# TJUMMG/OCPG

Measured on AMD Instinct MI355X. Metric: clips/sec fwd+bwd (5x384x640, R101), higher is better.
Workload: dtype bf16

## Files before the change

### include/ocpg_hip.h

```cpp
#ifndef OCPG_HIP_H
#define OCPG_HIP_H
#include <stdint.h>

#ifdef __cplusplus
extern "C" {
#endif

int ocpg_msda_fwd_f32(const float* value, const int64_t* shapes, const int64_t* level_start,
                      const float* loc, const float* attn,
                      int N, int S, int M, int D, int L, int Lq, int P,
                      float* out, const int64_t* shapes_host, void* stream);
int ocpg_msda_fwd_f64(const double* value, const int64_t* shapes, const int64_t* level_start,
                      const double* loc, const double* attn,
                      int N, int S, int M, int D, int L, int Lq, int P,
                      double* out, void* stream);

int ocpg_msda_bwd_f32(const float* value, const int64_t* shapes, const int64_t* level_start,
                      const float* loc, const float* attn, const float* grad_out,
                      int N, int S, int M, int D, int L, int Lq, int P,
                      float* grad_value, float* grad_loc, float* grad_attn,
                      const int64_t* shapes_host, void* stream);
int ocpg_msda_bwd_value_f32(const float* loc, const float* attn, const float* grad_out,
                            int N, int S, int M, int D, int L, int Lq, int P,
                            float* grad_value, const int64_t* shapes_host, void* stream);
// ... 6 lines not shown
                            int N, int S, int M, int D, int L, int Lq, int P,
                            float* out, float* loc_out, float* attn_out, void* stream);
int ocpg_msda_fused_bwd_qproj_f32(const float* value, const int64_t* shapes, const int64_t* level_start,
                                  const float* loc, const float* attn, const float* grad_out,
                                  int N, int S, int M, int D, int L, int Lq, int P,
                                  float* grad_qproj, void* stream);
int ocpg_msda_bwd_value_sel_f32(const float* loc, const float* attn, const float* grad_out,
                                int N, int S, int M, int D, int L, int Lq, int P,
                                float* grad_value, const int64_t* shapes_host, int* sel_state, void* stream);
int ocpg_msda_bwd_f64(const double* value, const int64_t* shapes, const int64_t* level_start,
                      const double* loc, const double* attn, const double* grad_out,
                      int N, int S, int M, int D, int L, int Lq, int P,
                      double* grad_value, double* grad_loc, double* grad_attn, void* stream);

int ocpg_bn_act_fwd(const void* x, const float* scale, const float* shift, const void* skip, void* y,
                    long long n_outer, int C, long long inner, int relu, int dtype, void* stream);
int ocpg_bn_act_bwd(const void* gy, const void* y, const float* scale, void* gx, void* gskip,
                    long long n_outer, int C, long long inner, int relu, int dtype, void* stream);

int ocpg_gemm_dgrad_bn_tile(long long M, int N, int K);
int ocpg_gemm_dgrad_bn(const void* a, const void* w, const void* c, const void* mask, const float* scale, void* out, void* out_skip,
                       long long M, int N, int K, int dtype, int tile, void* stream);

int ocpg_win_attn_fwd(const void* qkv, const float* biasT, const int* region, float scale, int BW, int NW, int N, int H,
                      int head_dim, void* out, float* lse, int dtype, void* stream);
int ocpg_win_attn_bwd(const void* qkv, const float* bias, const float* biasT, const int* region, float scale, int BW, int NW,
                      int N, int H, int head_dim, const void* out, const void* dout, const float* lse, void* dqkv, float* Dbuf,
                      float* dbiasT, int dtype, void* stream);

int ocpg_win_attn_bwd_mfma(const void* qkv, const float* bias, const float* biasT, const int* region, float scale, int BW, int NW, int N,
                           int H, int head_dim, const void* out, const void* dout, const float* lse, void* dqkv, float* Dbuf, void* dS,
                           int dtype, void* stream);

int ocpg_dynmask_fwd_f32(const float* feats, const float* params, const float* refpix, int BT, int Q, int C, int H, int W,
                         int stride, float* out, float* pre1, void* stream);

int ocpg_dynmask_bwd_pre_f32(const float* dout, const float* pre1, const float* params, int BT, int Q, int C, int H, int W,
                             int stride, float* dpre, float* part, float* w0d, void* stream);
int ocpg_dynmask_bwd_fin_f32(const float* part, const float* params, const float* refpix, const float* dw0, int BT, int Q, int C,
                             int H, int W, float* dparams, float* dref, void* stream);

int ocpg_im2col3x3_nhwc(const void* x, int N, int H, int W, int C, int stride, int dil, void* cols, int dtype, void* stream);
int ocpg_col2im3x3_nhwc(const void* dcols, int N, int H, int W, int C, int stride, int dil, void* dx, int dtype, void* stream);

int ocpg_conv3x3_mfma_fwd(const void* x, const void* w, const float* scale, const float* bias, int relu, int N, int H, int W,
                          int Cin, int Cout, int stride, void* y, void* stream);
// ... 169 lines not shown
```

### ocpg_amd/_lib.py

```python
import ctypes
import os

import torch

_HERE = os.path.dirname(os.path.abspath(__file__))
LIB_PATH = os.environ.get("OCPG_HIP_LIB") or os.path.join(_HERE, "lib", "libocpg_hip.so")
_lib = None

_i64p = ctypes.c_void_p
_vp = ctypes.c_void_p
_int = ctypes.c_int

SIGNATURES = {
    "ocpg_msda_fwd_f32": [_vp, _i64p, _i64p, _vp, _vp] + [_int] * 7 + [_vp, _vp, _vp],
    "ocpg_msda_fwd_f64": [_vp, _i64p, _i64p, _vp, _vp] + [_int] * 7 + [_vp, _vp],
    "ocpg_msda_bwd_f32": [_vp, _i64p, _i64p, _vp, _vp, _vp] + [_int] * 7 + [_vp, _vp, _vp, _vp, _vp],
    "ocpg_msda_bwd_value_f32": [_vp, _vp, _vp] + [_int] * 7 + [_vp, _vp, _vp],
    "ocpg_msda_fused_fwd_f32": [_vp, _i64p, _i64p, _vp, _vp] + [_int] * 7 + [_vp, _vp, _vp, _vp],
    "ocpg_msda_fused_bwd_qproj_f32": [_vp, _i64p, _i64p, _vp, _vp, _vp] + [_int] * 7 + [_vp, _vp],
    "ocpg_msda_bwd_value_sel_f32": [_vp, _vp, _vp] + [_int] * 7 + [_vp, _vp, _vp, _vp],
    "ocpg_msda_bwd_locattn_f32": [_vp, _i64p, _i64p, _vp, _vp, _vp] + [_int] * 7 + [_vp, _vp, _vp],
    "ocpg_msda_bwd_f64": [_vp, _i64p, _i64p, _vp, _vp, _vp] + [_int] * 7 + [_vp, _vp, _vp, _vp],
    "ocpg_bn_act_fwd": [_vp, _vp, _vp, _vp, _vp, ctypes.c_longlong, _int, ctypes.c_longlong, _int, _int, _vp],
    "ocpg_bn_act_bwd": [_vp, _vp, _vp, _vp, _vp, ctypes.c_longlong, _int, ctypes.c_longlong, _int, _int, _vp],
    "ocpg_gemm_dgrad_bn_tile": [ctypes.c_longlong, _int, _int],
    "ocpg_gemm_dgrad_bn": [_vp] * 7 + [ctypes.c_longlong, _int, _int, _int, _int, _vp],
    "ocpg_dynmask_fwd_f32": [_vp, _vp, _vp] + [_int] * 6 + [_vp, _vp, _vp],
    "ocpg_dynmask_bwd_pre_f32": [_vp, _vp, _vp] + [_int] * 6 + [_vp, _vp, _vp, _vp],
    "ocpg_dynmask_bwd_fin_f32": [_vp, _vp, _vp, _vp] + [_int] * 5 + [_vp, _vp, _vp],
    "ocpg_conv3x3_mfma_fwd": [_vp, _vp, _vp, _vp] + [_int] * 7 + [_vp, _vp],
    "ocpg_conv3x3_mfma_fwd_cols": [_vp, _vp, _vp, _vp] + [_int] * 7 + [_vp, _vp, _vp],
    "ocpg_conv3x3_mfma_dgrad": [_vp, _vp] + [_int] * 6 + [_vp, _vp],
    "ocpg_conv3x3_mfma_dgrad_masked": [_vp, _vp, _vp, _vp] + [_int] * 6 + [_vp, _vp],
    "ocpg_conv3x3_mfma_dgrad_w": [_vp, _vp, _vp, _vp] + [_int] * 6 + [_vp, _vp],
    "ocpg_conv3x3_mfma_splits": [_int] * 6,
    "ocpg_conv3x3_mfma_wgrad_splits": [_int] * 6,
    "ocpg_conv3x3_mfma_body_splits": [ctypes.c_longlong, _int, _int],
    "ocpg_conv3x3_mfma_fwd_bn_splitk": [_vp, _vp, _vp, _vp] + [_int] * 8 + [_vp, _vp, _vp],
    "ocpg_conv3x3_mfma_dgrad_w_splitk": [_vp, _vp, _vp, _vp] + [_int] * 7 + [_vp, _vp, _vp],
    "ocpg_conv3x3_mfma_wgrad": [_vp, _vp] + [_int] * 6 + [_vp, _vp],
    "ocpg_conv3x3_mfma_fwd_splitk": [_vp, _vp, _vp] + [_int] * 7 + [_vp, _vp, _int, _vp, _vp],
    "ocpg_gemm": [_vp, _vp, _vp, _vp] + [_int] * 4 + [ctypes.c_longlong] * 10 + [ctypes.c_float, ctypes.c_float, _vp],
    "ocpg_gemm_plans": [],
    "ocpg_gemm_tuned": [_vp],
    "ocpg_gemm_tune_rejected": [],
    "ocpg_gemm_set_tuning": [_int],
    "ocpg_gemm_export_picks": [_vp, ctypes.c_longlong],
    "ocpg_gemm_import_picks": [_vp, ctypes.c_longlong],
    "ocpg_window_means3x3_fwd": [_vp, ctypes.c_longlong, _int, _int, _int, _vp, _vp],
# ... 52 lines not shown
    "ocpg_colsum_partials": [_vp, ctypes.c_longlong, _int, _int, _vp, _vp],
    "ocpg_det_loss_fwd_f32": [_vp] * 7 + [ctypes.c_float] + [_int] * 5 + [_vp] * 3,
    "ocpg_det_loss_bwd_f32": [_vp] * 8 + [ctypes.c_float] + [_int] * 5 + [_vp] * 3,
    "ocpg_spectral_gate_fwd": [_vp] * 3 + [_int] * 3 + [_vp, _vp],
    "ocpg_spectral_gate_bwd": [_vp] * 4 + [_int] * 3 + [_vp, _vp, _vp],
    "ocpg_spectral_c2p": [_vp] * 3 + [_int] * 3 + [_vp, _int, _vp],
    "ocpg_spectral_p2c": [_vp] * 4 + [_int] * 3 + [_vp, _vp, _int, _vp],
    "ocpg_masked_ce_fwd_f32": [_vp] * 3 + [_int, ctypes.c_longlong, _vp, _vp],
    "ocpg_masked_ce_bwd_f32": [_vp] * 4 + [_int, ctypes.c_longlong, _vp, _vp],
    "ocpg_im2col3x3_nhwc": [_vp] + [_int] * 6 + [_vp, _int, _vp],
    "ocpg_col2im3x3_nhwc": [_vp] + [_int] * 6 + [_vp, _int, _vp],
    "ocpg_attn_smallk_fwd": [_vp, ctypes.c_longlong, _vp, ctypes.c_longlong, _vp, ctypes.c_longlong, _vp, ctypes.c_float] + [_int] * 5
                            + [ctypes.c_float, ctypes.c_ulonglong, ctypes.c_ulonglong, _vp, _vp, ctypes.c_longlong, _vp, _int, _vp],
    "ocpg_attn_smallk_bwd": [_vp, ctypes.c_longlong, _vp, ctypes.c_longlong, _vp, ctypes.c_longlong, _vp, _vp, ctypes.c_longlong, _vp,
                             ctypes.c_float] + [_int] * 5 + [ctypes.c_float, ctypes.c_ulonglong, ctypes.c_ulonglong, _vp, _vp, ctypes.c_longlong,
                                                             _vp, _vp, _int, _vp],
    "ocpg_win_attn_fwd": [_vp, _vp, _vp, ctypes.c_float] + [_int] * 5 + [_vp, _vp, _int, _vp],
    "ocpg_win_attn_bwd": [_vp, _vp, _vp, _vp, ctypes.c_float] + [_int] * 5 + [_vp] * 6 + [_int, _vp],
    "ocpg_win_attn_bwd_mfma": [_vp, _vp, _vp, _vp, ctypes.c_float] + [_int] * 5 + [_vp] * 6 + [_int, _vp],
}


_TIMING = {"on": False, "events": []}
_UNTIMED = ("ocpg_conv3x3_mfma_body_splits", "ocpg_gemm_dgrad_bn_tile", "ocpg_conv3x3_mfma_wgrad_splits", "ocpg_window_sums3x3_cl_bands", "ocpg_lfm_dft_supported", "ocpg_lfm_dft_split", "ocpg_conv3x3_mfma_splits", "ocpg_gemm_set_tuning", "ocpg_gemm_export_picks", "ocpg_gemm_import_picks", "ocpg_colsum_blocks", "ocpg_mso_wgrad_rows", "ocpg_gemm_plans", "ocpg_gemm_tuned", "ocpg_gemm_tune_rejected", "ocpg_bias_relu_dropout_bwd_slots", "ocpg_dropout_add_ln_bwd_slots", "ocpg_groupnorm_cl_work")


def enable_kernel_timing(on=True):
    _TIMING["on"] = on
    _TIMING["events"] = []


def collect_kernel_timing(work=None):
    torch.cuda.synchronize()
    out = {}
    for name, args, e0, e1 in _TIMING["events"]:
        d = out.setdefault(name, {"ms": 0.0, "n": 0, "work": 0.0, "modelled": 0})
        d["ms"] += e0.elapsed_time(e1)
        d["n"] += 1
        w = work(name, args) if work is not None else None
        if isinstance(w, tuple):
            d["work_lowp"] = d.get("work_lowp", 0.0) + (w[0] if w[1] else 0.0)
            w = w[0]
        if w is not None:
            d["work"] += w
            d["modelled"] += 1
    _TIMING["events"] = []
    _TIMING["on"] = False
# ... 39 lines not shown
        setattr(self, name, call)
        return call


def lib():
    global _lib
    if _lib is None:
        if not os.path.exists(LIB_PATH):
            raise RuntimeError(
                f"{LIB_PATH} not found: build it with `python -m ocpg_amd.csrc.build` "
                "(hipcc --offload-arch=gfx950). The HIP extension is mandatory; there is no CPU/PyTorch fallback.")
        L = ctypes.CDLL(LIB_PATH)
        for name, argtypes in SIGNATURES.items():
            fn = getattr(L, name)
            fn.argtypes = argtypes
            fn.restype = ctypes.c_int
        L.ocpg_hip_version.restype = ctypes.c_char_p
        L.ocpg_gemm_plans.restype = ctypes.c_longlong
        L.ocpg_gemm_tuned.restype = ctypes.c_longlong
        L.ocpg_gemm_tune_rejected.restype = ctypes.c_longlong
        L.ocpg_gemm_export_picks.restype = ctypes.c_longlong
        L.ocpg_gemm_set_tuning.restype = None
        L.ocpg_bias_relu_dropout_bwd_slots.restype = ctypes.c_longlong
        L.ocpg_dropout_add_ln_bwd_slots.restype = ctypes.c_longlong
        L.ocpg_groupnorm_cl_work.restype = ctypes.c_longlong
        L.ocpg_colsum_blocks.restype = ctypes.c_longlong
        _lib = _Lib(L)
    return _lib


def check(status, what):
    if status != 0:
        if status <= -1000:
            raise RuntimeError(f"{what}: invalid argument #{-status - 1000}")
        raise RuntimeError(f"{what}: HIP error {-status}")


def stream_ptr():
    return ctypes.c_void_p(torch.cuda.current_stream().cuda_stream)


def require_gpu(name, t):
    if not t.is_cuda:
        raise RuntimeError(f"{name} must be a GPU tensor: Not implemented on the CPU")
    if not t.is_contiguous():
        raise RuntimeError(f"{name} tensor has to be contiguous")
# ... 1 lines not shown
```

### ocpg_amd/csrc/fused_ln.hip

```cpp
#include <hip/hip_bf16.h>
#include <hip/hip_fp16.h>
#include <hip/hip_runtime.h>
#include <stdint.h>

#include "../../include/ocpg_hip.h"
#include "philox.h"

namespace {

using ocpg_dev::philox;

__device__ __forceinline__ void keep4(uint64_t seed, uint64_t offset, uint64_t idx4, uint32_t thr, float scale, float (&k)[4]) {
  if (thr == 0u) { k[0] = k[1] = k[2] = k[3] = 1.f; return; }
  const uint4 r = philox(make_uint2((uint32_t)seed, (uint32_t)(seed >> 32)),
                         make_uint4((uint32_t)idx4, (uint32_t)(idx4 >> 32), (uint32_t)offset, (uint32_t)(offset >> 32)));
  k[0] = r.x >= thr ? scale : 0.f; k[1] = r.y >= thr ? scale : 0.f; k[2] = r.z >= thr ? scale : 0.f; k[3] = r.w >= thr ? scale : 0.f;
}

template <typename T> struct IO;
template <> struct IO<float> {
  static __device__ __forceinline__ void load4(const float* p, float (&f)[4]) { const float4 v = *reinterpret_cast<const float4*>(p); f[0] = v.x; f[1] = v.y; f[2] = v.z; f[3] = v.w; }
  static __device__ __forceinline__ void store4(float* p, const float (&f)[4]) { *reinterpret_cast<float4*>(p) = make_float4(f[0], f[1], f[2], f[3]); }
};
template <> struct IO<__hip_bfloat16> {
  static __device__ __forceinline__ void load4(const __hip_bfloat16* p, float (&f)[4]) {
    const uint2 v = *reinterpret_cast<const uint2*>(p);
    f[0] = __uint_as_float(v.x << 16); f[1] = __uint_as_float(v.x & 0xffff0000u); f[2] = __uint_as_float(v.y << 16); f[3] = __uint_as_float(v.y & 0xffff0000u);
  }
  static __device__ __forceinline__ void store4(__hip_bfloat16* p, const float (&f)[4]) {
    uint32_t w[2];
#pragma unroll
    for (int i = 0; i < 2; ++i) {
      const __hip_bfloat16 lo = __float2bfloat16(f[2 * i]), hi = __float2bfloat16(f[2 * i + 1]);
      w[i] = (uint32_t)(*reinterpret_cast<const uint16_t*>(&lo)) | ((uint32_t)(*reinterpret_cast<const uint16_t*>(&hi)) << 16);
    }
    *reinterpret_cast<uint2*>(p) = make_uint2(w[0], w[1]);
  }
};

template <> struct IO<__half> {
// ... 199 lines not shown
  for (int g = g0; g < lpr; g += 256) {
    const int col = g * 4 * V;
    float acc[V][4];
#pragma unroll
    for (int v = 0; v < V; ++v)
#pragma unroll
      for (int j = 0; j < 4; ++j) acc[v][j] = 0.f;
    for (long long r = (long long)blockIdx.x * rpi + ro; r < R; r += (long long)gridDim.x * rpi) {
      float gv[V][4], hv[V][4], o[V][4];
      Wide<T, V>::load(gh + r * C + col, gv);
      Wide<T, V>::load(h + r * C + col, hv);
#pragma unroll
      for (int v = 0; v < V; ++v)
#pragma unroll
        for (int j = 0; j < 4; ++j) { o[v][j] = hv[v][j] > 0.f ? gv[v][j] * scale : 0.f; acc[v][j] += o[v][j]; }
      Wide<T, V>::store(ga + r * C + col, o);
    }
    float* o = dbias + ((long long)blockIdx.x * rpi + ro) * C + col;
#pragma unroll
    for (int v = 0; v < V; ++v) *reinterpret_cast<float4*>(o + 4 * v) = make_float4(acc[v][0], acc[v][1], acc[v][2], acc[v][3]);
  }
}

inline uint32_t threshold(float p) {
  if (p <= 0.f) return 0u;
  const double t = (double)p * 4294967296.0;
  return t >= 4294967295.0 ? 4294967295u : (uint32_t)t;
}

}

extern "C" {

int ocpg_dropout_add_ln_fwd(const void* x, const float* res, const float* gamma, const float* beta, long long R, int C, float eps, float p,
                            unsigned long long seed, unsigned long long offset, const unsigned long long* rng_base, int x_dtype, float* y,
                            float* mean, float* rstd, void* stream) {
  if (R < 0 || C <= 0 || C % 4 != 0 || C > 64 * 4 * NCH_MAX) return -1006;
  if (p < 0.f || p >= 1.f) return -1007;
  if (R == 0) return 0;
  if (!x || !res || !gamma || !beta) return -1001;
  if (!y || !mean || !rstd) return -1010;
  const uint32_t thr = threshold(p);
  const float scale = 1.f / (1.f - p);
  const unsigned grid = (unsigned)((R + 3) / 4);
  hipStream_t st = (hipStream_t)stream;
  if (x_dtype < 0 || x_dtype > 2) return -1008;
  const int nc = (C + 255) / 256;
#define DAL_FWD(XT_, N_) dal_fwd<XT_, N_><<<grid, 256, 0, st>>>((const XT_*)x, res, gamma, beta, R, C, eps, thr, scale, seed, offset, (const uint64_t*)rng_base, y, mean, rstd)
#define DAL_FWD_T(XT_) do { if (nc <= 1) DAL_FWD(XT_, 1); else if (nc <= 2) DAL_FWD(XT_, 2); else if (nc <= 4) DAL_FWD(XT_, 4); else DAL_FWD(XT_, 8); } while (0)
  if (x_dtype == 0) DAL_FWD_T(float); else if (x_dtype == 1) DAL_FWD_T(__hip_bfloat16); else DAL_FWD_T(__half);
  const hipError_t e = hipGetLastError();
// ... 90 lines not shown
```

### ocpg_amd/csrc/philox.h

```cpp
#pragma once
#include <hip/hip_runtime.h>
#include <stdint.h>

namespace ocpg_dev {

__device__ __forceinline__ uint4 philox(uint2 key, uint4 c) {
#pragma unroll
  for (int r = 0; r < 10; ++r) {
    const uint32_t lo0 = 0xD2511F53u * c.x, hi0 = __umulhi(0xD2511F53u, c.x);
    const uint32_t lo1 = 0xCD9E8D57u * c.z, hi1 = __umulhi(0xCD9E8D57u, c.z);
    c = make_uint4(hi1 ^ c.y ^ key.x, lo1, hi0 ^ c.w ^ key.y, lo0);
    key.x += 0x9E3779B9u;
    key.y += 0xBB67AE85u;
  }
  return c;
}

}
```

### ocpg_amd/models/deformable_transformer.py

```python
import copy

import torch
import torch.nn.functional as F
from torch import nn

from ..util.misc import fully_valid, inverse_sigmoid, mask_key, memo
from . import amp_cache
from .attention import MultiheadAttention
from .ops.functions import fused_ln_func
from .ops.modules import MSDeformAttn

FUSED_GLUE = True


def _drop_add_norm(x, res, drop, norm):
    if FUSED_GLUE and isinstance(norm, nn.LayerNorm) and norm.elementwise_affine and fused_ln_func.supported(x, res, x.shape[-1]):
        return fused_ln_func.dropout_add_layer_norm(x, res, norm, drop.p if drop.training else 0.0)
    return norm(res + drop(x))


def _ffn_hidden(src, linear1, activation, drop):
    if FUSED_GLUE and activation is F.relu and src.is_cuda and linear1.bias is not None:
        w, b = amp_cache.lookup(linear1.weight), amp_cache.lookup(linear1.bias)
        x = src
        if torch.is_autocast_enabled("cuda"):
            dt = torch.get_autocast_dtype("cuda")
            x, w, b = x.to(dt), w.to(dt), b.to(dt)
        if x.dtype == w.dtype and x.dtype in (torch.float32, torch.bfloat16, torch.float16) and w.shape[0] % 4 == 0:
            x2 = x.reshape(-1, x.shape[-1])
            splits = amp_cache._split_rows(x2.shape[0]) if amp_cache.SPLIT_K else 1
            h = fused_ln_func.LinearBiasReluDropout.apply(x2, w, b, drop.p if drop.training else 0.0, None, splits)
            return h.view(*x.shape[:-1], w.shape[0])
    return drop(activation(linear1(src)))


def _clones(module, n):
    out = []
    for _ in range(n):
        c = copy.deepcopy(module)
        for p, q in zip(module.parameters(), c.parameters()):
            if getattr(p, "_ocpg_single_use", False):
                q._ocpg_single_use = True
        out.append(c)
    return nn.ModuleList(out)


def _activation(name):
    if name == "relu":
        return F.relu
    if name == "gelu":
        return F.gelu
    if name == "glu":
        return F.glu
    raise RuntimeError(f"activation should be relu/gelu, not {name}.")


class DeformableTransformerEncoderLayer(nn.Module):
    def __init__(self, d_model=256, d_ffn=1024, dropout=0.1, activation="relu", n_levels=4, n_heads=8, n_points=4):
        super().__init__()
        self.self_attn = MSDeformAttn(d_model, n_levels, n_heads, n_points)
        self.dropout1 = nn.Dropout(dropout)
        self.norm1 = nn.LayerNorm(d_model)
        self.linear1 = amp_cache.Linear(d_model, d_ffn)
        amp_cache.mark_single_use(self.linear1)
        self.activation = _activation(activation)
        self.dropout2 = nn.Dropout(dropout)
        self.linear2 = amp_cache.Linear(d_ffn, d_model)
        amp_cache.mark_single_use(self.linear2)
        self.dropout3 = nn.Dropout(dropout)
        self.norm2 = nn.LayerNorm(d_model)

    def forward(self, src, pos, reference_points, spatial_shapes, level_start_index, padding_mask=None):
        with torch.autocast(device_type=src.device.type, enabled=False):
            q = src.float() if pos is None else src.float() + pos.float()
            attn = self.self_attn(q, reference_points, src.float(), spatial_shapes, level_start_index, padding_mask)[0]
        src = _drop_add_norm(attn, src, self.dropout1, self.norm1)
        ffn = self.linear2(_ffn_hidden(src, self.linear1, self.activation, self.dropout2))
        return _drop_add_norm(ffn, src, self.dropout3, self.norm2)


class DeformableTransformerEncoder(nn.Module):
    def __init__(self, encoder_layer, num_layers):
        super().__init__()
        self.layers = _clones(encoder_layer, num_layers)
        self.num_layers = num_layers

    @staticmethod
    def get_reference_points(spatial_shapes, valid_ratios, device):
        host = getattr(spatial_shapes, "_ocpg_host", None)
        shapes = host.tolist() if host is not None else spatial_shapes.tolist()
        per_level = []
        for lvl, (h, w) in enumerate(shapes):
            ys = torch.linspace(0.5, h - 0.5, h, dtype=torch.float32, device=device)
            xs = torch.linspace(0.5, w - 0.5, w, dtype=torch.float32, device=device)
            gy, gx = torch.meshgrid(ys, xs, indexing="ij")
            gy = gy.reshape(-1)[None] / (valid_ratios[:, None, lvl, 1] * h)
            gx = gx.reshape(-1)[None] / (valid_ratios[:, None, lvl, 0] * w)
            per_level.append(torch.stack((gx, gy), -1))
        ref = torch.cat(per_level, 1)
        return ref[:, :, None] * valid_ratios[:, None]
# ... 13 lines not shown
        self.cross_attn = MSDeformAttn(d_model, n_levels, n_heads, n_points)
        self.dropout1 = nn.Dropout(dropout)
        self.norm1 = nn.LayerNorm(d_model)
        self.self_attn = MultiheadAttention(d_model, n_heads, dropout=dropout)
        self.dropout2 = nn.Dropout(dropout)
        self.norm2 = nn.LayerNorm(d_model)
        self.linear1 = amp_cache.Linear(d_model, d_ffn)
        amp_cache.mark_single_use(self.linear1)
        self.activation = _activation(activation)
        self.dropout3 = nn.Dropout(dropout)
        self.linear2 = amp_cache.Linear(d_ffn, d_model)
        amp_cache.mark_single_use(self.linear2)
        self.dropout4 = nn.Dropout(dropout)
        self.norm3 = nn.LayerNorm(d_model)

    def forward(self, tgt, query_pos, reference_points, src, src_spatial_shapes, level_start_index, src_padding_mask=None):
        qk = tgt if query_pos is None else tgt + query_pos
        sa = self.self_attn(qk.transpose(0, 1), qk.transpose(0, 1), tgt.transpose(0, 1)).transpose(0, 1)
        tgt = _drop_add_norm(sa, tgt, self.dropout2, self.norm2)
        with torch.autocast(device_type=tgt.device.type, enabled=False):
            q = tgt.float() if query_pos is None else tgt.float() + query_pos.float()
            ca, loc, weights = self.cross_attn(q, reference_points, src.float(), src_spatial_shapes, level_start_index, src_padding_mask)
        tgt = _drop_add_norm(ca, tgt, self.dropout1, self.norm1)
        ffn = self.linear2(_ffn_hidden(tgt, self.linear1, self.activation, self.dropout3))
        return _drop_add_norm(ffn, tgt, self.dropout4, self.norm3), loc, weights


class DeformableTransformerDecoder(nn.Module):
    TOPK_SAMPLES = 30

    def __init__(self, decoder_layer, num_layers, return_intermediate=False):
        super().__init__()
        self.layers = _clones(decoder_layer, num_layers)
        self.num_layers = num_layers
        self.return_intermediate = return_intermediate
        self.compute_samples = True
        self.bbox_embed = None
        self.class_embed = None

    def forward(self, tgt, reference_points, src, src_spatial_shapes, src_level_start_index, src_valid_ratios,
                query_pos=None, src_padding_mask=None):
        out = tgt
        inter, inter_refs, inter_samples = [], [], []
        self.box_deltas = [] if self.bbox_embed is not None else None
        samples_keep = None
        for lid, layer in enumerate(self.layers):
            if reference_points.shape[-1] == 4:
# ... 144 lines not shown
```

### ocpg_amd/models/ops/functions/fused_ln_func.py

```python
import torch
from torch.autograd import Function
from torch.autograd.function import once_differentiable

from ...._lib import check, lib
from .gemm_func import mm

_DT = {torch.float32: 0, torch.bfloat16: 1, torch.float16: 2}
_calls = [0]
_active = [None]


class GraphRng:

    def __init__(self, device):
        self.state = torch.zeros(2, dtype=torch.int64, device=device)
        self.c0, self.calls = None, 0

    def __enter__(self):
        assert _active[0] is None, "nested graph captures of the dropout generator"
        self.c0 = _calls[0]
        _active[0] = self
        return self

    def __exit__(self, *exc):
        self.calls = _calls[0] - self.c0
        _calls[0] = self.c0
        _active[0] = None
        return False

    def advance(self):
# ... 43 lines not shown
              "ocpg_dropout_add_ln_fwd")
        ctx.save_for_backward(x2, res2, gamma, stats)
        ctx.meta = (float(p), seed, offset, base, x.shape, res.shape)
        return y.view(res.shape)

    @staticmethod
    @once_differentiable
    def backward(ctx, gy):
        x2, res2, gamma, stats = ctx.saved_tensors
        p, seed, offset, base, xshape, rshape = ctx.meta
        r, c = x2.shape
        gy = gy.reshape(r, c).float().contiguous()
        gx = torch.empty_like(x2) if ctx.needs_input_grad[0] else None
        gres = torch.empty_like(res2) if ctx.needs_input_grad[1] else None
        part = torch.empty((lib().ocpg_dropout_add_ln_bwd_slots(r), 2, c), dtype=torch.float32, device=x2.device)
        check(lib().ocpg_dropout_add_ln_bwd(gy.data_ptr(), x2.data_ptr(), res2.data_ptr(), gamma.data_ptr(), stats[0].data_ptr(), stats[1].data_ptr(),
                                            r, c, p, seed, offset, base, _DT[x2.dtype], None if gx is None else gx.data_ptr(),
                                            None if gres is None else gres.data_ptr(), part.data_ptr(), _st()),
              "ocpg_dropout_add_ln_bwd")
        dgb = part.sum(0)
        return (None if gx is None else gx.view(xshape), None if gres is None else gres.view(rshape), dgb[0], dgb[1], None, None, None)


class LinearBiasReluDropout(Function):
    @staticmethod
    def forward(ctx, x2, w, b, p, rng, splits):
        seed, offset, base = _unpack(rng)
        h = mm(x2, w, True)
        r, c = h.shape
        check(lib().ocpg_bias_relu_dropout_fwd(h.data_ptr(), b.data_ptr(), r, c, float(p), seed, offset, base, _DT[h.dtype], h.data_ptr(), _st()),
              "ocpg_bias_relu_dropout_fwd")
        ctx.save_for_backward(x2, w, h)
        ctx.meta = (float(p), splits)
        from ...amp_cache import deferrable
        ctx.defer_w, ctx.defer_b = deferrable(w), deferrable(b) and b.dtype == h.dtype
        return h

    @staticmethod
    @once_differentiable
    def backward(ctx, gh):
        from ...amp_cache import weight_grad
        x2, w, h = ctx.saved_tensors
        p, splits = ctx.meta
        r, c = h.shape
        gh = gh.to(h.dtype).contiguous()
        ga = torch.empty_like(h)
        slots = lib().ocpg_bias_relu_dropout_bwd_slots(r, c, _DT[h.dtype])
        part = torch.empty((slots, c), dtype=torch.float32, device=h.device)
        check(lib().ocpg_bias_relu_dropout_bwd(gh.data_ptr(), h.data_ptr(), r, c, p, _DT[h.dtype], ga.data_ptr(), part.data_ptr(), _st()),
              "ocpg_bias_relu_dropout_bwd")
        from ...amp_cache import defer_sum
        dbias = defer_sum(part, h.dtype) if (ctx.defer_b and ctx.needs_input_grad[2] and h.dtype != torch.float32) else part.sum(0).to(h.dtype)
        gx = mm(ga, w) if ctx.needs_input_grad[0] else None
        gw = weight_grad(ga, x2, ctx.defer_w) if ctx.needs_input_grad[1] else None
        return gx, gw, dbias if ctx.needs_input_grad[2] else None, None, None, None


def supported(x, res, c):
    return (x.is_cuda and x.dtype in _DT and res.dtype == torch.float32 and c % 4 == 0 and c <= 2048 and x.shape == res.shape)


def dropout_add_layer_norm(x, res, norm, p, rng=None):
    return DropoutAddLayerNorm.apply(x, res, norm.weight, norm.bias, p, norm.eps, rng)
```

Measured before the change: 60.14.

## Fuse FFN linear1 GEMM with bias-ReLU-dropout epilogue in forward and backward

Adds a bf16 MFMA GEMM kernel for K=256 transformer FFNs. In the forward pass it applies bias, ReLU and Philox dropout in the epilogue. In the backward pass it multiplies gy by w2 and applies the ReLU/dropout mask while producing per-panel bias-gradient partials. A new FeedForward autograd function wires both kernels into the encoder and decoder layers and falls back to the existing path when the shape or dtype is declined. This removes the intermediate writes and re-reads of the hidden activation and the separate elementwise kernels, at the cost of a hand-written GEMM that may be slower than the tuned library GEMM.

Measured after the change: 60.95, median of 6. 1.4% higher.

```diff
diff --git a/include/ocpg_hip.h b/include/ocpg_hip.h
--- a/include/ocpg_hip.h
+++ b/include/ocpg_hip.h
@@ -52,6 +52,12 @@
 int ocpg_gemm_dgrad_bn(const void* a, const void* w, const void* c, const void* mask, const float* scale, void* out, void* out_skip,
                        long long M, int N, int K, int dtype, int tile, void* stream);
 
+int ocpg_ffn_gemm_fwd(const void* x, const void* w1, const void* b1, void* h, long long M, int N, int K, float p, unsigned long long seed,
+                      unsigned long long offset, const unsigned long long* rng_base, int dtype, int nsplit, void* stream);
+long long ocpg_ffn_gemm_bwd_slots(long long M, int N);
+int ocpg_ffn_gemm_bwd(const void* gy, const void* w2, const void* h, void* ga, float* dbias_part, long long M, int N, int K, float p,
+                      int dtype, int nsplit, void* stream);
+
 int ocpg_win_attn_fwd(const void* qkv, const float* biasT, const int* region, float scale, int BW, int NW, int N, int H,
                       int head_dim, void* out, float* lse, int dtype, void* stream);
 int ocpg_win_attn_bwd(const void* qkv, const float* bias, const float* biasT, const int* region, float scale, int BW, int NW,
diff --git a/ocpg_amd/_lib.py b/ocpg_amd/_lib.py
--- a/ocpg_amd/_lib.py
+++ b/ocpg_amd/_lib.py
@@ -25,6 +25,9 @@
     "ocpg_bn_act_bwd": [_vp, _vp, _vp, _vp, _vp, ctypes.c_longlong, _int, ctypes.c_longlong, _int, _int, _vp],
     "ocpg_gemm_dgrad_bn_tile": [ctypes.c_longlong, _int, _int],
     "ocpg_gemm_dgrad_bn": [_vp] * 7 + [ctypes.c_longlong, _int, _int, _int, _int, _vp],
+    "ocpg_ffn_gemm_fwd": [_vp] * 4 + [ctypes.c_longlong, _int, _int, ctypes.c_float, ctypes.c_ulonglong, ctypes.c_ulonglong, _vp, _int, _int, _vp],
+    "ocpg_ffn_gemm_bwd_slots": [ctypes.c_longlong, _int],
+    "ocpg_ffn_gemm_bwd": [_vp] * 5 + [ctypes.c_longlong, _int, _int, ctypes.c_float, _int, _int, _vp],
     "ocpg_dynmask_fwd_f32": [_vp, _vp, _vp] + [_int] * 6 + [_vp, _vp, _vp],
     "ocpg_dynmask_bwd_pre_f32": [_vp, _vp, _vp] + [_int] * 6 + [_vp, _vp, _vp, _vp],
     "ocpg_dynmask_bwd_fin_f32": [_vp, _vp, _vp, _vp] + [_int] * 5 + [_vp, _vp, _vp],
@@ -123,7 +126,7 @@
 
 
 _TIMING = {"on": False, "events": []}
-_UNTIMED = ("ocpg_conv3x3_mfma_body_splits", "ocpg_gemm_dgrad_bn_tile", "ocpg_conv3x3_mfma_wgrad_splits", "ocpg_window_sums3x3_cl_bands", "ocpg_lfm_dft_supported", "ocpg_lfm_dft_split", "ocpg_conv3x3_mfma_splits", "ocpg_gemm_set_tuning", "ocpg_gemm_export_picks", "ocpg_gemm_import_picks", "ocpg_colsum_blocks", "ocpg_mso_wgrad_rows", "ocpg_gemm_plans", "ocpg_gemm_tuned", "ocpg_gemm_tune_rejected", "ocpg_bias_relu_dropout_bwd_slots", "ocpg_dropout_add_ln_bwd_slots", "ocpg_groupnorm_cl_work")
+_UNTIMED = ("ocpg_conv3x3_mfma_body_splits", "ocpg_gemm_dgrad_bn_tile", "ocpg_ffn_gemm_bwd_slots", "ocpg_conv3x3_mfma_wgrad_splits", "ocpg_window_sums3x3_cl_bands", "ocpg_lfm_dft_supported", "ocpg_lfm_dft_split", "ocpg_conv3x3_mfma_splits", "ocpg_gemm_set_tuning", "ocpg_gemm_export_picks", "ocpg_gemm_import_picks", "ocpg_colsum_blocks", "ocpg_mso_wgrad_rows", "ocpg_gemm_plans", "ocpg_gemm_tuned", "ocpg_gemm_tune_rejected", "ocpg_bias_relu_dropout_bwd_slots", "ocpg_dropout_add_ln_bwd_slots", "ocpg_groupnorm_cl_work")
 
 
 def enable_kernel_timing(on=True):
@@ -209,6 +212,7 @@
         L.ocpg_gemm_export_picks.restype = ctypes.c_longlong
         L.ocpg_gemm_set_tuning.restype = None
         L.ocpg_bias_relu_dropout_bwd_slots.restype = ctypes.c_longlong
+        L.ocpg_ffn_gemm_bwd_slots.restype = ctypes.c_longlong
         L.ocpg_dropout_add_ln_bwd_slots.restype = ctypes.c_longlong
         L.ocpg_groupnorm_cl_work.restype = ctypes.c_longlong
         L.ocpg_colsum_blocks.restype = ctypes.c_longlong
diff --git a/ocpg_amd/csrc/fused_ln.hip b/ocpg_amd/csrc/fused_ln.hip
--- a/ocpg_amd/csrc/fused_ln.hip
+++ b/ocpg_amd/csrc/fused_ln.hip
@@ -8,14 +8,8 @@
 
 namespace {
 
+using ocpg_dev::keep4;
 using ocpg_dev::philox;
-
-__device__ __forceinline__ void keep4(uint64_t seed, uint64_t offset, uint64_t idx4, uint32_t thr, float scale, float (&k)[4]) {
-  if (thr == 0u) { k[0] = k[1] = k[2] = k[3] = 1.f; return; }
-  const uint4 r = philox(make_uint2((uint32_t)seed, (uint32_t)(seed >> 32)),
-                         make_uint4((uint32_t)idx4, (uint32_t)(idx4 >> 32), (uint32_t)offset, (uint32_t)(offset >> 32)));
-  k[0] = r.x >= thr ? scale : 0.f; k[1] = r.y >= thr ? scale : 0.f; k[2] = r.z >= thr ? scale : 0.f; k[3] = r.w >= thr ? scale : 0.f;
-}
 
 template <typename T> struct IO;
 template <> struct IO<float> {
@@ -261,11 +255,7 @@
   }
 }
 
-inline uint32_t threshold(float p) {
-  if (p <= 0.f) return 0u;
-  const double t = (double)p * 4294967296.0;
-  return t >= 4294967295.0 ? 4294967295u : (uint32_t)t;
-}
+inline uint32_t threshold(float p) { return ocpg_dev::dropout_threshold(p); }
 
 }
 
diff --git a/ocpg_amd/csrc/gemm_ffn.hip b/ocpg_amd/csrc/gemm_ffn.hip
--- /dev/null
+++ b/ocpg_amd/csrc/gemm_ffn.hip
@@ -0,0 +1,296 @@
+#include <hip/hip_bf16.h>
+#include <hip/hip_runtime.h>
+#include <stdint.h>
+
+#include "../../include/ocpg_hip.h"
+#include "philox.h"
+
+namespace {
+
+using ocpg_dev::philox_wide;
+
+typedef short bf16x8 __attribute__((ext_vector_type(8)));
+typedef short s4 __attribute__((ext_vector_type(4)));
+typedef float f32x16 __attribute__((ext_vector_type(16)));
+typedef unsigned u32x4 __attribute__((ext_vector_type(4)));
+
+constexpr int KP = 256;
+constexpr int TM = 64, TN = 64, NT = 256;
+constexpr int PLD = KP + 8;
+constexpr int BLD = TN + 8;
+constexpr int T_L = 64 * KP / 8 / NT;
+
+constexpr int DECLINE_SHAPE = -2000, DECLINE_ALIGN = -2001, DECLINE_DTYPE = -2002;
+
+__device__ __forceinline__ void unpack8(const u32x4 u, float (&f)[8]) {
+#pragma unroll
+  for (int i = 0; i < 4; ++i) {
+    f[2 * i] = __uint_as_float(u[i] << 16);
+    f[2 * i + 1] = __uint_as_float(u[i] & 0xffff0000u);
+  }
+}
+
+__device__ __forceinline__ uint4 pack8(const float (&f)[8]) {
+  uint32_t w[4];
+#pragma unroll
+  for (int i = 0; i < 4; ++i)
+    w[i] = (uint32_t)__bfloat16_as_ushort(__float2bfloat16(f[2 * i])) | ((uint32_t)__bfloat16_as_ushort(__float2bfloat16(f[2 * i + 1])) << 16);
+  return make_uint4(w[0], w[1], w[2], w[3]);
+}
+
+struct Args {
+  const __hip_bfloat16* a;
+  const __hip_bfloat16* w;
+  const __hip_bfloat16* bias;
+  const __hip_bfloat16* h;
+  __hip_bfloat16* out;
+  float* dbias;
+  const uint64_t* rng_base;
+  uint64_t seed, offset;
+  uint32_t thr;
+  float scale;
+  long long M;
+  int N;
+};
+
+template <bool BWD, bool FULL>
+__device__ __forceinline__ void ffn_walk(const Args& g, short* __restrict__ Ap, short* __restrict__ Bs, short* __restrict__ St, float (*Cs)[TN]) {
+  constexpr int WLD = BWD ? BLD : PLD;
+  const int tid = threadIdx.x, lane = tid & 63, wave = tid >> 6;
+  const int wm = wave & 1, wn = wave >> 1;
+  const long long M = g.M, m0 = (long long)blockIdx.x * TM;
+  const int N = g.N;
+  const int tiles = (N / TN) / (int)gridDim.y, j0 = (int)blockIdx.y * tiles;
+  const int prow = tid >> 5, pseg = tid & 31, srow = tid >> 3, sseg = tid & 7;
+
+  auto fetch = [&](u32x4 (&R)[T_L], int t) __attribute__((always_inline)) {
+    const int n0 = (j0 + min(t, tiles - 1)) * TN;
+#pragma unroll
+    for (int i = 0; i < T_L; ++i) {
+      const __hip_bfloat16* p = BWD ? g.w + (long long)(srow + 32 * i) * N + n0 + sseg * 8 : g.w + (long long)(n0 + prow + 8 * i) * KP + pseg * 8;
+      R[i] = *reinterpret_cast<const u32x4*>(p);
+    }
+  };
+  auto park = [&](const u32x4 (&R)[T_L]) __attribute__((always_inline)) {
+#pragma unroll
+    for (int i = 0; i < T_L; ++i)
+      *reinterpret_cast<u32x4*>(BWD ? &Bs[(srow + 32 * i) * WLD + sseg * 8] : &Bs[(prow + 8 * i) * WLD + pseg * 8]) = R[i];
+  };
+
+  const int erow = tid >> 3, c8 = (tid & 7) * 8;
+  const bool ok0 = FULL || m0 + erow < M, ok1 = FULL || m0 + erow + 32 < M;
+  const long long eoff = (m0 + erow) * N + c8;
+  const uint64_t offset = g.offset + (g.rng_base ? *g.rng_base : 0ull);
+  u32x4 preA[2] = {{0u, 0u, 0u, 0u}, {0u, 0u, 0u, 0u}}, preB[2] = {{0u, 0u, 0u, 0u}, {0u, 0u, 0u, 0u}};
+  auto preload = [&](u32x4 (&pre)[2], int t) __attribute__((always_inline)) {
+    const int n0 = (j0 + min(t, tiles - 1)) * TN;
+    if (BWD) {
+      if (ok0) pre[0] = *reinterpret_cast<const u32x4*>(g.h + eoff + n0);
+      if (ok1) pre[1] = *reinterpret_cast<const u32x4*>(g.h + eoff + n0 + 32ll * N);
+    } else {
+      pre[0] = *reinterpret_cast<const u32x4*>(g.bias + n0 + c8);
+    }
+  };
+
+  u32x4 RT[T_L];
+  fetch(RT, 0);
+  {
+    u32x4 P[T_L];
+#pragma unroll
+    for (int i = 0; i < T_L; ++i) P[i] = *reinterpret_cast<const u32x4*>(g.a + (FULL ? m0 + prow + 8 * i : min(m0 + prow + 8 * i, M - 1)) * KP + pseg * 8);
+#pragma unroll
+    for (int i = 0; i < T_L; ++i) *reinterpret_cast<u32x4*>(&Ap[(prow + 8 * i) * PLD + pseg * 8]) = P[i];
+  }
+  park(RT);
+  preload(preA, 0);
+  preload(preB, 1);
+  fetch(RT, 1);
+
+  const int fr = lane & 31, fh = lane >> 5;
+  auto btr = [&](int k0, int ncol0) __attribute__((always_inline)) -> bf16x8 {
+    const int li = lane & 15, grp = lane >> 4;
+    const short* p = &Bs[(k0 + 8 * fh + (li >> 2)) * WLD + ncol0 + 16 * (grp & 1) + 4 * (li & 3)];
+    const s4 lo = __builtin_amdgcn_ds_read_tr16_b64_v4i16((__attribute__((address_space(3))) s4*)p);
+    const s4 hi = __builtin_amdgcn_ds_read_tr16_b64_v4i16((__attribute__((address_space(3))) s4*)(p + 4 * WLD));
+    bf16x8 r;
+    r[0] = lo[0]; r[1] = lo[1]; r[2] = lo[2]; r[3] = lo[3]; r[4] = hi[0]; r[5] = hi[1]; r[6] = hi[2]; r[7] = hi[3];
+    return r;
+  };
+  auto flush = [&](int t) __attribute__((always_inline)) {
+    if (BWD && tid < TN)
+      g.dbias[(long long)blockIdx.x * N + (j0 + t) * TN + tid] = ((Cs[0][tid] + Cs[1][tid]) + Cs[2][tid]) + Cs[3][tid];
+  };
+
+  u32x4 sv0, sv1;
+  auto mma_tile = [&](int t) __attribute__((always_inline)) {
+    f32x16 acc;
+#pragma unroll
+    for (int r = 0; r < 16; ++r) acc[r] = 0.f;
+#pragma unroll
+    for (int ks = 0; ks < KP / 16; ++ks) {
+      const bf16x8 af = *reinterpret_cast<const bf16x8*>(&Ap[(wm * 32 + fr) * PLD + ks * 16 + fh * 8]);
+      bf16x8 bf;
+      if (BWD) bf = btr(ks * 16, wn * 32);
+      else bf = *reinterpret_cast<const bf16x8*>(&Bs[(wn * 32 + fr) * WLD + ks * 16 + fh * 8]);
+      acc = __builtin_amdgcn_mfma_f32_32x32x16_bf16(af, bf, acc, 0, 0, 0);
+    }
+    short* st0 = St + (wm * 32 + 4 * fh) * BLD + wn * 32 + fr;
+#pragma unroll
+    for (int r = 0; r < 16; ++r) st0[((r & 3) + 8 * (r >> 2)) * BLD] = (short)__bfloat16_as_ushort(__float2bfloat16(acc[r]));
+    __syncthreads();
+    if (t > 0) flush(t - 1);
+    park(RT);
+    fetch(RT, t + 2);
+    sv0 = *reinterpret_cast<const u32x4*>(&St[erow * BLD + c8]);
+    sv1 = *reinterpret_cast<const u32x4*>(&St[(erow + 32) * BLD + c8]);
+    __syncthreads();
+  };
+  auto epilogue = [&](int t, u32x4 (&pre)[2]) __attribute__((always_inline)) {
+    const int n0 = (j0 + t) * TN;
+    float v[2][8];
+    unpack8(sv0, v[0]);
+    unpack8(sv1, v[1]);
+    if (BWD) {
+      float cs[8];
+#pragma unroll
+      for (int q = 0; q < 2; ++q) {
+        float hv[8];
+        unpack8(pre[q], hv);
+#pragma unroll
+        for (int i = 0; i < 8; ++i) v[q][i] = ((q ? ok1 : ok0) && hv[i] > 0.f) ? v[q][i] * g.scale : 0.f;
+      }
+#pragma unroll
+      for (int i = 0; i < 8; ++i) cs[i] = v[0][i] + v[1][i];
+      __builtin_amdgcn_sched_barrier(0);
+      preload(pre, t + 2);
+      if (ok0) *reinterpret_cast<uint4*>(g.out + eoff + n0) = pack8(v[0]);
+      if (ok1) *reinterpret_cast<uint4*>(g.out + eoff + n0 + 32ll * N) = pack8(v[1]);
+#pragma unroll
+      for (int i = 0; i < 8; ++i) {
+        cs[i] += __shfl_xor(cs[i], 8);
+        cs[i] += __shfl_xor(cs[i], 16);
+        cs[i] += __shfl_xor(cs[i], 32);
+      }
+      if (lane < 8) {
+        *reinterpret_cast<float4*>(&Cs[wave][c8]) = make_float4(cs[0], cs[1], cs[2], cs[3]);
+        *reinterpret_cast<float4*>(&Cs[wave][c8 + 4]) = make_float4(cs[4], cs[5], cs[6], cs[7]);
+      }
+    } else {
+      float bv[8];
+      unpack8(pre[0], bv);
+      __builtin_amdgcn_sched_barrier(0);
+      preload(pre, t + 2);
+#pragma unroll
+      for (int q = 0; q < 2; ++q) {
+        const long long off = eoff + n0 + (q ? 32ll * N : 0ll);
+        float k[8] = {1.f, 1.f, 1.f, 1.f, 1.f, 1.f, 1.f, 1.f};
+        if (g.thr != 0u) {
+          const uint2 key = make_uint2((uint32_t)g.seed, (uint32_t)(g.seed >> 32));
+          const uint64_t i4 = (uint64_t)off / 4;
+          const uint4 r0 = philox_wide(key, make_uint4((uint32_t)i4, (uint32_t)(i4 >> 32), (uint32_t)offset, (uint32_t)(offset >> 32)));
+          const uint4 r1 = philox_wide(key, make_uint4((uint32_t)(i4 + 1), (uint32_t)((i4 + 1) >> 32), (uint32_t)offset, (uint32_t)(offset >> 32)));
+          const uint32_t r[8] = {r0.x, r0.y, r0.z, r0.w, r1.x, r1.y, r1.z, r1.w};
+#pragma unroll
+          for (int i = 0; i < 8; ++i) k[i] = r[i] >= g.thr ? g.scale : 0.f;
+        }
+#pragma unroll
+        for (int i = 0; i < 8; ++i) v[q][i] = fmaxf(v[q][i] + bv[i], 0.f) * k[i];
+        if (q ? ok1 : ok0) *reinterpret_cast<uint4*>(g.out + off) = pack8(v[q]);
+      }
+    }
+  };
+
+  __syncthreads();
+  mma_tile(0);
+  for (int t = 0;; t += 2) {
+    epilogue(t, preA);
+    if (t + 1 == tiles) break;
+    mma_tile(t + 1);
+    epilogue(t + 1, preB);
+    if (t + 2 == tiles) break;
+    mma_tile(t + 2);
+  }
+  if (BWD) {
+    __syncthreads();
+    flush(tiles - 1);
+  }
+}
+
+template <bool BWD>
+__global__ __launch_bounds__(NT) void gemm_ffn(const Args g) {
+  __shared__ __attribute__((aligned(16))) short Ap[TM * PLD];
+  __shared__ __attribute__((aligned(16))) short Bs[BWD ? KP * BLD : TN * PLD];
+  __shared__ __attribute__((aligned(16))) short St[TM * BLD];
+  __shared__ float Cs[BWD ? 4 : 1][TN];
+  if ((long long)(blockIdx.x + 1) * TM <= g.M) ffn_walk<BWD, true>(g, Ap, Bs, St, Cs);
+  else ffn_walk<BWD, false>(g, Ap, Bs, St, Cs);
+}
+
+inline bool aligned16(const void* p) { return ((uintptr_t)p & 15u) == 0; }
+
+inline int pick_split(long long M, int N, int nsplit) {
+  const int ntiles = N / TN;
+  if (nsplit > 0) return ntiles % nsplit == 0 ? nsplit : -1;
+  const long long panels = (M + TM - 1) / TM;
+  int s = 1;
+  while (panels * s < 2048 && ntiles % (2 * s) == 0 && ntiles / (2 * s) >= 4) s *= 2;
+  return s;
+}
+
+inline int check_shape(long long M, int N, int K, int dtype, int nsplit) {
+  if (dtype != 1) return DECLINE_DTYPE;
+  if (M < 0 || N <= 0 || K <= 0) return -1007;
+  if (K != KP || N % TN != 0 || (M + TM - 1) / TM > 0x7fffffffll) return DECLINE_SHAPE;
+  if (nsplit < 0 || pick_split(M, N, nsplit) < 0) return -1013;
+  return 0;
+}
+
+}
+
+extern "C" int ocpg_ffn_gemm_fwd(const void* x, const void* w1, const void* b1, void* h, long long M, int N, int K, float p,
+                                 unsigned long long seed, unsigned long long offset, const unsigned long long* rng_base, int dtype, int nsplit,
+                                 void* stream) {
+  const int rc = check_shape(M, N, K, dtype, nsplit);
+  if (rc) return rc;
+  if (p < 0.f || p >= 1.f) return -1008;
+  if (!x) return -1001;
+  if (!w1) return -1002;
+  if (!b1) return -1003;
+  if (!h) return -1004;
+  if (!aligned16(x) || !aligned16(w1) || !aligned16(b1) || !aligned16(h) || ((uintptr_t)rng_base & 7u)) return DECLINE_ALIGN;
+  if (M == 0) return 0;
+  Args g{};
+  g.a = (const __hip_bfloat16*)x, g.w = (const __hip_bfloat16*)w1, g.bias = (const __hip_bfloat16*)b1, g.out = (__hip_bfloat16*)h;
+  g.rng_base = (const uint64_t*)rng_base, g.seed = seed, g.offset = offset;
+  g.thr = ocpg_dev::dropout_threshold(p), g.scale = 1.f / (1.f - p), g.M = M, g.N = N;
+  const dim3 grid((unsigned)((M + TM - 1) / TM), (unsigned)pick_split(M, N, nsplit));
+  gemm_ffn<false><<<grid, NT, 0, (hipStream_t)stream>>>(g);
+  const hipError_t err = hipGetLastError();
+  return err == hipSuccess ? 0 : -(int)err;
+}
+
+extern "C" long long ocpg_ffn_gemm_bwd_slots(long long M, int N) {
+  if (M <= 0 || N <= 0 || N % TN != 0) return 0;
+  return (M + TM - 1) / TM;
+}
+
+extern "C" int ocpg_ffn_gemm_bwd(const void* gy, const void* w2, const void* h, void* ga, float* dbias_part, long long M, int N, int K, float p,
+                                 int dtype, int nsplit, void* stream) {
+  const int rc = check_shape(M, N, K, dtype, nsplit);
+  if (rc) return rc;
+  if (p < 0.f || p >= 1.f) return -1009;
+  if (!gy) return -1001;
+  if (!w2) return -1002;
+  if (!h) return -1003;
+  if (!ga) return -1004;
+  if (!dbias_part) return -1005;
+  if (!aligned16(gy) || !aligned16(w2) || !aligned16(h) || !aligned16(ga) || !aligned16(dbias_part)) return DECLINE_ALIGN;
+  if (M == 0) return 0;
+  Args g{};
+  g.a = (const __hip_bfloat16*)gy, g.w = (const __hip_bfloat16*)w2, g.h = (const __hip_bfloat16*)h, g.out = (__hip_bfloat16*)ga;
+  g.dbias = dbias_part, g.scale = 1.f / (1.f - p), g.M = M, g.N = N;
+  const dim3 grid((unsigned)((M + TM - 1) / TM), (unsigned)pick_split(M, N, nsplit));
+  gemm_ffn<true><<<grid, NT, 0, (hipStream_t)stream>>>(g);
+  const hipError_t err = hipGetLastError();
+  return err == hipSuccess ? 0 : -(int)err;
+}
diff --git a/ocpg_amd/csrc/philox.h b/ocpg_amd/csrc/philox.h
--- a/ocpg_amd/csrc/philox.h
+++ b/ocpg_amd/csrc/philox.h
@@ -16,4 +16,28 @@
   return c;
 }
 
+__device__ __forceinline__ uint4 philox_wide(uint2 key, uint4 c) {
+#pragma unroll
+  for (int r = 0; r < 10; ++r) {
+    const uint64_t p0 = (uint64_t)0xD2511F53u * c.x, p1 = (uint64_t)0xCD9E8D57u * c.z;
+    c = make_uint4((uint32_t)(p1 >> 32) ^ c.y ^ key.x, (uint32_t)p1, (uint32_t)(p0 >> 32) ^ c.w ^ key.y, (uint32_t)p0);
+    key.x += 0x9E3779B9u;
+    key.y += 0xBB67AE85u;
+  }
+  return c;
 }
+
+__device__ __forceinline__ void keep4(uint64_t seed, uint64_t offset, uint64_t idx4, uint32_t thr, float scale, float (&k)[4]) {
+  if (thr == 0u) { k[0] = k[1] = k[2] = k[3] = 1.f; return; }
+  const uint4 r = philox(make_uint2((uint32_t)seed, (uint32_t)(seed >> 32)),
+                         make_uint4((uint32_t)idx4, (uint32_t)(idx4 >> 32), (uint32_t)offset, (uint32_t)(offset >> 32)));
+  k[0] = r.x >= thr ? scale : 0.f; k[1] = r.y >= thr ? scale : 0.f; k[2] = r.z >= thr ? scale : 0.f; k[3] = r.w >= thr ? scale : 0.f;
+}
+
+inline uint32_t dropout_threshold(float p) {
+  if (p <= 0.f) return 0u;
+  const double t = (double)p * 4294967296.0;
+  return t >= 4294967295.0 ? 4294967295u : (uint32_t)t;
+}
+
+}
diff --git a/ocpg_amd/models/deformable_transformer.py b/ocpg_amd/models/deformable_transformer.py
--- a/ocpg_amd/models/deformable_transformer.py
+++ b/ocpg_amd/models/deformable_transformer.py
@@ -34,6 +34,20 @@
     return drop(activation(linear1(src)))
 
 
+def _ffn(src, linear1, activation, drop, linear2):
+    if (FUSED_GLUE and fused_ln_func.FUSED_FFN and amp_cache.SPLIT_K and activation is F.relu and src.is_cuda and torch.is_grad_enabled()
+            and linear1.bias is not None and linear2.bias is not None and torch.is_autocast_enabled("cuda")
+            and torch.get_autocast_dtype("cuda") == torch.bfloat16 and src.shape[-1] == 256 and linear1.weight.shape[0] % 64 == 0
+            and src.numel() >= 256 * max(fused_ln_func.FFN_MIN_ROWS, amp_cache.TOKEN_LINEAR_MIN_ROWS)):
+        w1, b1, w2, b2 = (amp_cache.lookup(t) for t in (linear1.weight, linear1.bias, linear2.weight, linear2.bias))
+        if w2.requires_grad:
+            dt = torch.bfloat16
+            x2 = src.to(dt).reshape(-1, 256)
+            y = fused_ln_func.FeedForward.apply(x2, w1.to(dt), b1.to(dt), w2.to(dt), b2.to(dt), drop.p if drop.training else 0.0, None)
+            return y.view(*src.shape[:-1], w2.shape[0])
+    return linear2(_ffn_hidden(src, linear1, activation, drop))
+
+
 def _clones(module, n):
     out = []
     for _ in range(n):
@@ -75,7 +89,7 @@
             q = src.float() if pos is None else src.float() + pos.float()
             attn = self.self_attn(q, reference_points, src.float(), spatial_shapes, level_start_index, padding_mask)[0]
         src = _drop_add_norm(attn, src, self.dropout1, self.norm1)
-        ffn = self.linear2(_ffn_hidden(src, self.linear1, self.activation, self.dropout2))
+        ffn = _ffn(src, self.linear1, self.activation, self.dropout2, self.linear2)
         return _drop_add_norm(ffn, src, self.dropout3, self.norm2)
 
 
@@ -135,7 +149,7 @@
             q = tgt.float() if query_pos is None else tgt.float() + query_pos.float()
             ca, loc, weights = self.cross_attn(q, reference_points, src.float(), src_spatial_shapes, level_start_index, src_padding_mask)
         tgt = _drop_add_norm(ca, tgt, self.dropout1, self.norm1)
-        ffn = self.linear2(_ffn_hidden(tgt, self.linear1, self.activation, self.dropout3))
+        ffn = _ffn(tgt, self.linear1, self.activation, self.dropout3, self.linear2)
         return _drop_add_norm(ffn, tgt, self.dropout4, self.norm3), loc, weights
 
 
diff --git a/ocpg_amd/models/ops/functions/fused_ln_func.py b/ocpg_amd/models/ops/functions/fused_ln_func.py
--- a/ocpg_amd/models/ops/functions/fused_ln_func.py
+++ b/ocpg_amd/models/ops/functions/fused_ln_func.py
@@ -1,3 +1,5 @@
+import os
+
 import torch
 from torch.autograd import Function
 from torch.autograd.function import once_differentiable
@@ -6,6 +8,9 @@
 from .gemm_func import mm
 
 _DT = {torch.float32: 0, torch.bfloat16: 1, torch.float16: 2}
+FUSED_FFN = os.environ.get("OCPG_FUSED_FFN", "1") != "0"
+FFN_MIN_ROWS = 4096
+_FFN_DECLINED = (-2000, -2001, -2002)
 _calls = [0]
 _active = [None]
 
@@ -95,14 +100,48 @@
         return (None if gx is None else gx.view(xshape), None if gres is None else gres.view(rshape), dgb[0], dgb[1], None, None, None)
 
 
+def _ffn_eligible(x2, w):
+    return (FUSED_FFN and x2.dtype == torch.bfloat16 and w.dtype == torch.bfloat16 and x2.dim() == 2 and x2.shape[0] >= FFN_MIN_ROWS
+            and x2.is_contiguous() and w.is_contiguous())
+
+
+def _hidden_fwd(x2, w, b, p, seed, offset, base):
+    if _ffn_eligible(x2, w) and b.dtype == x2.dtype and b.is_contiguous():
+        r, c = x2.shape[0], w.shape[0]
+        h = torch.empty((r, c), dtype=x2.dtype, device=x2.device)
+        rc = lib().ocpg_ffn_gemm_fwd(x2.data_ptr(), w.data_ptr(), b.data_ptr(), h.data_ptr(), r, c, x2.shape[1], float(p), seed, offset, base,
+                                     _DT[h.dtype], 0, _st())
+        if rc == 0:
+            return h
+        if rc not in _FFN_DECLINED:
+            check(rc, "ocpg_ffn_gemm_fwd")
+    h = mm(x2, w, True)
+    r, c = h.shape
+    check(lib().ocpg_bias_relu_dropout_fwd(h.data_ptr(), b.data_ptr(), r, c, float(p), seed, offset, base, _DT[h.dtype], h.data_ptr(), _st()),
+          "ocpg_bias_relu_dropout_fwd")
+    return h
+
+
+def _hidden_bwd(gh, h, p):
+    r, c = h.shape
+    ga = torch.empty_like(h)
+    slots = lib().ocpg_bias_relu_dropout_bwd_slots(r, c, _DT[h.dtype])
+    part = torch.empty((slots, c), dtype=torch.float32, device=h.device)
+    check(lib().ocpg_bias_relu_dropout_bwd(gh.data_ptr(), h.data_ptr(), r, c, p, _DT[h.dtype], ga.data_ptr(), part.data_ptr(), _st()),
+          "ocpg_bias_relu_dropout_bwd")
+    return ga, part
+
+
+def _bias_grad(part, dtype, defer):
+    from ...amp_cache import defer_sum
+    return defer_sum(part, dtype) if (defer and dtype != torch.float32) else part.sum(0).to(dtype)
+
+
 class LinearBiasReluDropout(Function):
     @staticmethod
     def forward(ctx, x2, w, b, p, rng, splits):
         seed, offset, base = _unpack(rng)
-        h = mm(x2, w, True)
-        r, c = h.shape
-        check(lib().ocpg_bias_relu_dropout_fwd(h.data_ptr(), b.data_ptr(), r, c, float(p), seed, offset, base, _DT[h.dtype], h.data_ptr(), _st()),
-              "ocpg_bias_relu_dropout_fwd")
+        h = _hidden_fwd(x2, w, b, p, seed, offset, base)
         ctx.save_for_backward(x2, w, h)
         ctx.meta = (float(p), splits)
         from ...amp_cache import deferrable
@@ -115,20 +154,55 @@
         from ...amp_cache import weight_grad
         x2, w, h = ctx.saved_tensors
         p, splits = ctx.meta
-        r, c = h.shape
         gh = gh.to(h.dtype).contiguous()
-        ga = torch.empty_like(h)
-        slots = lib().ocpg_bias_relu_dropout_bwd_slots(r, c, _DT[h.dtype])
-        part = torch.empty((slots, c), dtype=torch.float32, device=h.device)
-        check(lib().ocpg_bias_relu_dropout_bwd(gh.data_ptr(), h.data_ptr(), r, c, p, _DT[h.dtype], ga.data_ptr(), part.data_ptr(), _st()),
-              "ocpg_bias_relu_dropout_bwd")
-        from ...amp_cache import defer_sum
-        dbias = defer_sum(part, h.dtype) if (ctx.defer_b and ctx.needs_input_grad[2] and h.dtype != torch.float32) else part.sum(0).to(h.dtype)
+        ga, part = _hidden_bwd(gh, h, p)
+        dbias = _bias_grad(part, h.dtype, ctx.defer_b and ctx.needs_input_grad[2])
         gx = mm(ga, w) if ctx.needs_input_grad[0] else None
         gw = weight_grad(ga, x2, ctx.defer_w) if ctx.needs_input_grad[1] else None
         return gx, gw, dbias if ctx.needs_input_grad[2] else None, None, None, None
 
 
+class FeedForward(Function):
+
+    @staticmethod
+    def forward(ctx, x2, w1, b1, w2, b2, p, rng):
+        from ...amp_cache import deferrable
+        seed, offset, base = _unpack(rng)
+        h = _hidden_fwd(x2, w1, b1, p, seed, offset, base)
+        ctx.save_for_backward(x2, w1, h, w2)
+        ctx.p = float(p)
+        ctx.defer_w1, ctx.defer_b1 = deferrable(w1), deferrable(b1) and b1.dtype == h.dtype
+        ctx.defer_w2, ctx.defer_b2 = deferrable(w2), b2 if deferrable(b2) else None
+        return mm(h, w2, True, b2)
+
+    @staticmethod
+    @once_differentiable
+    def backward(ctx, gy):
+        from ...amp_cache import colsum, weight_grad
+        x2, w1, h, w2 = ctx.saved_tensors
+        p = ctx.p
+        r, c = h.shape
+        gy = gy.to(h.dtype).contiguous()
+        ga = part = None
+        if _ffn_eligible(gy, w2):
+            ga = torch.empty_like(h)
+            part = torch.empty((max(int(lib().ocpg_ffn_gemm_bwd_slots(r, c)), 1), c), dtype=torch.float32, device=h.device)
+            rc = lib().ocpg_ffn_gemm_bwd(gy.data_ptr(), w2.data_ptr(), h.data_ptr(), ga.data_ptr(), part.data_ptr(), r, c, gy.shape[1], p,
+                                         _DT[h.dtype], 0, _st())
+            if rc in _FFN_DECLINED:
+                ga = part = None
+            elif rc:
+                check(rc, "ocpg_ffn_gemm_bwd")
+        if ga is None:
+            ga, part = _hidden_bwd(mm(gy, w2), h, p)
+        gw2 = weight_grad(gy, h, ctx.defer_w2) if ctx.needs_input_grad[3] else None
+        gb2 = colsum(gy, ctx.defer_b2) if ctx.needs_input_grad[4] else None
+        db1 = _bias_grad(part, h.dtype, ctx.defer_b1) if ctx.needs_input_grad[2] else None
+        gx = mm(ga, w1) if ctx.needs_input_grad[0] else None
+        gw1 = weight_grad(ga, x2, ctx.defer_w1) if ctx.needs_input_grad[1] else None
+        return gx, gw1, db1, gw2, gb2, None, None
+
+
 def supported(x, res, c):
     return (x.is_cuda and x.dtype in _DT and res.dtype == torch.float32 and c % 4 == 0 and c <= 2048 and x.shape == res.shape)
 
```
